# iSEE-Laboratory/DiffuVolume

Measured on AMD Instinct MI355X. Metric: stereo pairs/sec, SceneFlow 960x540 (cropped 960x512) maxdisp=192, hot path, higher is better.
Workload: dtype f32; 1 GPU; SceneFlow ACVNet+DiffuVolume hot path (gwc + concat*softmax(att) + 5 DDIM steps + EPE), 960x512, maxdisp=192, batch=8/GPU, random-init weights; global_batch=8, ddim_steps=5, parallelism=dp1

## Files before the change

### diffuvolume_amd/csrc/conv3d_s2pp.hip

```cpp

#include <atomic>
#include <type_traits>

#include "dv_common.h"

namespace {

typedef float f32x2 __attribute__((ext_vector_type(2)));

constexpr int kPPLoaders = 3;
constexpr int kPPDepth = 3;

template <int SHAPE_>
struct PG {
  static constexpr int SHAPE = SHAPE_;
  static_assert(SHAPE == 0 || SHAPE == 1, "patch shapes");
  static constexpr int TR = SHAPE == 0 ? 2 : 4, TC = 16 / TR;
  static constexpr int KC = 4, NT = 2, TD = 2;
  static constexpr int IZ = 2 * TD + 1, IY = 4 * TR + 1;
  static constexpr int LQ = SHAPE == 0 ? TC + 2 : TC + 1;
  static constexpr int RX = SHAPE == 0 ? 40 : 20;
  static constexpr int ROWS = IZ * IY;
  static constexpr int CS = ROWS * RX;
  static constexpr int QPC = ROWS * LQ;
  static constexpr int NQ = KC * QPC;
  static constexpr int NP = (NQ + 63) / 64;
  static constexpr int RAW_FLOATS = ((NP + 3) / 4 * 4) * 256;
  static_assert(RX == 4 * LQ && CS == 4 * QPC, "the loaded quads of a chunk are contiguous in LDS: quad `it` at float 4 * it");
  static_assert(4 * RAW_FLOATS * 4 <= 160 * 1024, "one block per CU: two sub-tiles x two bricks");
};

namespace pp {
constexpr int U_CHUNK = 3 * 4 * 4 * 4 * 16 * 4;
__host__ __device__ constexpr int amap(int i) { return i < 2 ? 0 : (i == 2 ? 1 : 2); }
__host__ __device__ constexpr int bmap(int i) { return i == 3 ? 1 : (i == 4 ? 3 : i); }
}

struct PPArgs {
  const float* in;
  const float* wpk;
  const float* ch_scale;
  const float* ch_bias;
  const float* residual;
  float* out;
  int B, Cin, D, H, W, Cout, Do, Ho, Wo;
  int ntx, nty, ntz, nco;
  int ntiles;
  int act;
  int vec_ok;
  unsigned wpk_bytes;
};

struct Tile { int tcb, z0, y0, x0, b; bool valid; };

template <int SHAPE>
__global__ __launch_bounds__(512 + 64 * kPPLoaders, 1) void conv3d_s2pp_kernel(PPArgs a) {
  using G = PG<SHAPE>;
  constexpr int KC = G::KC, NT = G::NT, TR = G::TR, TC = G::TC, IY = G::IY, RX = G::RX, CS = G::CS, LQ = G::LQ;
  constexpr int NQ = G::NQ, QPC = G::QPC, NP = G::NP, RAW_FLOATS = G::RAW_FLOATS;
  __shared__ __attribute__((aligned(16))) float raw_a0[RAW_FLOATS];
  __shared__ __attribute__((aligned(16))) float raw_b0[RAW_FLOATS];
  __shared__ __attribute__((aligned(16))) float raw_a1[RAW_FLOATS];
  __shared__ __attribute__((aligned(16))) float raw_b1[RAW_FLOATS];

  const int tid = threadIdx.x;
  const int lane = tid & 63;
  const int wave = __builtin_amdgcn_readfirstlane(tid >> 6);

  const unsigned nblk = gridDim.x, xcd = blockIdx.x & 7u, bidx = blockIdx.x >> 3;
  const unsigned nbx = (nblk >> 3) + (xcd < (nblk & 7u) ? 1u : 0u);
  const unsigned npairs = ((unsigned)a.ntiles + 1u) >> 1;
  const unsigned tq = npairs >> 3, trm = npairs & 7u;
  const unsigned slab_lo = xcd < trm ? xcd * (tq + 1) : trm * (tq + 1) + (xcd - trm) * tq;
  const unsigned slab_n = tq + (xcd < trm ? 1u : 0u);
  const int my_tiles = __builtin_amdgcn_readfirstlane(bidx < slab_n ? (int)((slab_n - bidx + nbx - 1) / nbx) : 0);
  if (my_tiles == 0) return;

  auto tile_at = [&](int k, int h) __attribute__((always_inline)) {
    unsigned t = 2u * (slab_lo + bidx + (unsigned)k * nbx) + (unsigned)h;
    Tile r;
    r.valid = t < (unsigned)a.ntiles;
    if (!r.valid) t = (unsigned)a.ntiles - 1u;
    r.tcb = t % a.nco; t /= a.nco;
    r.x0 = (t % a.ntx) * 2 * TC; t /= a.ntx;
    r.y0 = (t % a.nty) * 2 * TR; t /= a.nty;
    r.z0 = (t % a.ntz) * G::TD;
    r.b = t / a.ntz;
    return r;
  };

  const size_t plane = (size_t)a.H * a.W;
  const size_t vol = (size_t)a.D * plane;
  const unsigned vol_bytes = (unsigned)__builtin_amdgcn_readfirstlane((int)(vol * sizeof(float)));
  const int n_chunk = (a.Cin + KC - 1) / KC;
  const int NCH = (n_chunk + 1) & ~1;
  const bool share = (a.nco & 1) == 0;
  const int n_steps = my_tiles * NCH;

  if (wave >= 8) {
    constexpr int NL = kPPLoaders, NPL = (NP + NL - 1) / NL;
    const int li = wave - 8;
    static_assert(NL * NPL * 256 <= RAW_FLOATS, "every piece a loader writes lies inside the buffer");
    unsigned sob0[NPL], sob1[NPL];
    auto plan = [&](const Tile& t, unsigned (&sob)[NPL]) __attribute__((always_inline)) {
#pragma unroll
      for (int p = 0; p < NPL; ++p) {
        const int it = 64 * (li + NL * p) + lane;
        const int cl = it / QPC, r1 = it - cl * QPC;
        const int row = r1 / LQ, q = r1 - row * LQ;
        const int zz = row / IY, yy = row - zz * IY;
        const int z = 2 * t.z0 - 1 + zz, y = 2 * t.y0 - 1 + yy, x = 2 * t.x0 - 4 + 4 * q;
        const bool ok = t.valid && it < NQ && (unsigned)z < (unsigned)a.D && (unsigned)y < (unsigned)a.H &&
                        (unsigned)x < (unsigned)a.W;
        sob[p] = ok ? (unsigned)cl * vol_bytes + (unsigned)((z * a.H + y) * a.W + x) * 4u : 0xfffffff0u;
      }
    };
    auto dma_raw = [&](const Tile& t, const unsigned (&sob)[NPL], int c, float* dst) __attribute__((always_inline)) {
      const int c0 = c * KC;
      const int left = a.Cin - c0;
      const unsigned rec = left <= 0 ? 0u : (unsigned)(left < KC ? left : KC) * vol_bytes;
      const uint64_t ba = reinterpret_cast<uint64_t>(a.in + ((size_t)t.b * a.Cin + (left > 0 ? c0 : 0)) * vol);
      const uint64_t bu = (uint64_t)(unsigned)__builtin_amdgcn_readfirstlane((int)(unsigned)ba) |
                          ((uint64_t)(unsigned)__builtin_amdgcn_readfirstlane((int)(unsigned)(ba >> 32)) << 32);
      const auto rs = __builtin_amdgcn_make_buffer_rsrc(reinterpret_cast<float*>(bu), 0,
                                                        __builtin_amdgcn_readfirstlane((int)rec), 0x00020000);
#pragma unroll
      for (int p = 0; p < NPL; ++p)
        __builtin_amdgcn_raw_ptr_buffer_load_lds(rs, (__attribute__((address_space(3))) void*)(dst + (li + NL * p) * 256), 16,
                                                 (int)sob[p], 0, 0, 0);
    };
    Tile ft0 = tile_at(0, 0), ft1 = tile_at(0, 1);
    int fk = 0, fc = 0;
    auto advance = [&]() __attribute__((always_inline)) {
      if (++fc == NCH) {
        fc = 0;
        if (++fk < my_tiles) { ft0 = tile_at(fk, 0); ft1 = tile_at(fk, 1); plan(ft0, sob0); plan(ft1, sob1); }
      }
    };
    auto fetch = [&](float* d0, float* d1) __attribute__((always_inline)) {
      dma_raw(ft0, sob0, fc, d0);
      if (!share) dma_raw(ft1, sob1, fc, d1);
      advance();
    };
    plan(ft0, sob0);
    plan(ft1, sob1);
    fetch(raw_a0, raw_a1);
    fetch(raw_b0, raw_b1);
    auto arrive = [&]() __attribute__((always_inline)) {
      asm volatile("s_waitcnt vmcnt(0)" ::: "memory");
      __syncthreads();
    };
    arrive();
#pragma unroll 1
    for (int s = 0; s < n_steps; s += 2) {
      arrive();
      if (s + 2 < n_steps) fetch(raw_a0, raw_a1);
      arrive();
      if (s + 3 < n_steps) fetch(raw_b0, raw_b1);
    }
    return;
  }

  const int sub = wave >> 2, pl = (wave >> 1) & 1, nh = wave & 1;
  const int j = lane & 15, kq = lane >> 4;
  const float* const raw_a = (sub && !share) ? raw_a1 : raw_a0;
  const float* const raw_b = (sub && !share) ? raw_b1 : raw_b0;

  const uint64_t wb = reinterpret_cast<uint64_t>(a.wpk);
  const uint64_t wbs = (uint64_t)(unsigned)__builtin_amdgcn_readfirstlane((int)(unsigned)wb) |
                       ((uint64_t)(unsigned)__builtin_amdgcn_readfirstlane((int)(unsigned)(wb >> 32)) << 32);
  const auto wrs = __builtin_amdgcn_make_buffer_rsrc(reinterpret_cast<float*>(wbs), 0, (int)a.wpk_bytes, 0x00020000);
  const int wvoff = lane * 16;
  constexpr int PD = kPPDepth, RD = PD == 5 ? 6 : PD + 1;
  static_assert(12 % RD == 0, "ring slots repeat with the step");
  f32x4 bq[RD][NT];
  auto load_b = [&](int tcb, int chunk, int g, int slot) __attribute__((always_inline)) {
    const int ch = chunk < n_chunk ? chunk : n_chunk - 1;
    const int kd = g >> 2, by = g & 3;
    const int base = (ch * a.nco + tcb) * (pp::U_CHUNK * 4);
#pragma unroll
    for (int n = 0; n < NT; ++n) {
      const int so = base + (((kd * 4 + 2 * nh + n) * 4 + by) * 256) * 4;
      bq[slot][n] = __builtin_bit_cast(f32x4, __builtin_amdgcn_raw_buffer_load_b128(wrs, wvoff, so, 0));
    }
  };

  const int a_tr = j / TC, a_tc = j % TC;
  const int patch_lo = kq * CS + ((2 * pl) * IY + 4 * a_tr) * RX + 4 * a_tc;

  float V[2][5][5];
  auto read_row = [&](const float* rb, int kd, int slot, int r) __attribute__((always_inline)) {
    const float* p = rb + patch_lo + kd * IY * RX;
    V[slot][r][0] = p[r * RX + 3];
    const f32x4 qd = *reinterpret_cast<const f32x4*>(p + r * RX + 4);
    V[slot][r][1] = qd[0]; V[slot][r][2] = qd[1]; V[slot][r][3] = qd[2]; V[slot][r][4] = qd[3];
  };
  auto col_tf = [&](int slot, int r) __attribute__((always_inline)) {
    V[slot][r][0] -= V[slot][r][2];
    V[slot][r][4] -= V[slot][r][2];
  };
  auto row_tf = [&](int slot) __attribute__((always_inline)) {
#pragma unroll
    for (int c = 0; c < 5; ++c) {
      V[slot][0][c] -= V[slot][2][c];
      V[slot][4][c] -= V[slot][2][c];
    }
  };

  f32x4 acc[3][3][NT];
  auto zero_acc = [&]() __attribute__((always_inline)) {
#pragma unroll
    for (int i = 0; i < 3; ++i)
#pragma unroll
      for (int jj = 0; jj < 3; ++jj)
#pragma unroll
        for (int n = 0; n < NT; ++n) acc[i][jj][n] = (f32x4){0.f, 0.f, 0.f, 0.f};
  };

  const size_t oplane = (size_t)a.Ho * a.Wo;
  const float slope = a.act == DV_ACT_RELU ? 0.f : (a.act == DV_ACT_LEAKY ? 0.01f : 1.f);
  auto epilogue = [&](const Tile& t) __attribute__((always_inline)) {
    constexpr int RL = TC < 4 ? TC : 4, NRUN = 4 / RL;
    const int zo = t.z0 + pl;
    if (zo >= a.Do || !t.valid) return;
    const bool fast = a.vec_ok && t.x0 + 2 * TC <= a.Wo && t.y0 + 2 * TR <= a.Ho;
#pragma unroll
    for (int n = 0; n < NT; ++n) {
      const int co = t.tcb * 64 + nh * 32 + n * 16 + j;
      if (co >= a.Cout) continue;
      const float sc = a.ch_scale ? a.ch_scale[co] : 1.f;
      const float bi = a.ch_bias ? a.ch_bias[co] : 0.f;
      const size_t cbase = (((size_t)t.b * a.Cout + co) * a.Do + zo) * oplane;
#pragma unroll
      for (int run = 0; run < NRUN; ++run) {
        const int m0 = 4 * kq + run * RL;
        const int yo = t.y0 + 2 * (m0 / TC), xo = t.x0 + 2 * (m0 % TC);
#pragma unroll
        for (int ya = 0; ya < 2; ++ya) {
          float v[2 * RL];
#pragma unroll
          for (int e = 0; e < RL; ++e)
#pragma unroll
            for (int xb = 0; xb < 2; ++xb) {
              const int ee = run * RL + e;
              v[2 * e + xb] = (acc[ya][xb][n][ee] + acc[ya][xb + 1][n][ee]) + (acc[ya + 1][xb][n][ee] + acc[ya + 1][xb + 1][n][ee]);
            }
          const size_t o = cbase + (size_t)(yo + ya) * a.Wo + xo;
          if (fast) {
#pragma unroll
            for (int h = 0; h < RL / 2; ++h) {
              f32x4 u = (f32x4){v[4 * h], v[4 * h + 1], v[4 * h + 2], v[4 * h + 3]} * sc + bi;
              if (a.residual) u += *reinterpret_cast<const f32x4*>(a.residual + o + 4 * h);
              if (a.act == DV_ACT_MISH) {
#pragma unroll
                for (int e = 0; e < 4; ++e) u[e] = dv_act(u[e], DV_ACT_MISH);
              } else {
                u = __builtin_elementwise_max(u, u * slope);
              }
              *reinterpret_cast<f32x4*>(a.out + o + 4 * h) = u;
            }
          } else if (yo + ya < a.Ho) {
#pragma unroll
            for (int e = 0; e < 2 * RL; ++e)
              if (xo + e < a.Wo) {
                float u = fmaf(v[e], sc, bi);
                if (a.residual) u += a.residual[o + e];
                a.out[o + e] = dv_act(u, a.act);
              }
          }
        }
      }
    }
  };

  Tile cur = tile_at(0, sub);
  Tile nxt = my_tiles > 1 ? tile_at(1, sub) : cur;
#pragma unroll
  for (int g = 0; g < PD; ++g) load_b(cur.tcb, 0, g, g);
  zero_acc();
  __syncthreads();
#pragma unroll
  for (int r = 0; r < 5; ++r) read_row(raw_a, 0, 0, r);
  row_tf(0);
  col_tf(0, 0); col_tf(0, 2); col_tf(0, 4);

  auto step = [&](int c, auto parity) __attribute__((always_inline)) {
    constexpr int PAR = decltype(parity)::value;
    const float* rb = PAR ? raw_b : raw_a;
    const float* nb = PAR ? raw_a : raw_b;
    const bool n1 = c + 1 >= NCH;
    const int c1 = n1 ? 0 : c + 1;
    const int tcb1 = n1 ? nxt.tcb : cur.tcb;
#pragma unroll
    for (int g = 0; g < 12; ++g) {
      const int kd = g >> 2, by = g & 3;
      const int slot = (PAR + kd) & 1, nslot = slot ^ 1;
      if (g == 10) __syncthreads();
      if (g + PD < 12) load_b(cur.tcb, c, g + PD, (g + PD) % RD);
      else load_b(tcb1, c1, g + PD - 12, (g + PD) % RD);
      {
        const float* src = kd < 2 ? rb : nb;
        const int nkd = kd < 2 ? kd + 1 : 0;
        if (by == 0) { col_tf(slot, 1); col_tf(slot, 3); }
        if (by == 2) { read_row(src, nkd, nslot, 0); read_row(src, nkd, nslot, 2); read_row(src, nkd, nslot, 4); }
        if (by == 3) { read_row(src, nkd, nslot, 1); read_row(src, nkd, nslot, 3); }
      }
#pragma unroll
      for (int i = 0; i < 5; ++i) {
        if (pp::bmap(i) != by) continue;
#pragma unroll
        for (int jj = 0; jj < 5; ++jj)
#pragma unroll
          for (int n = 0; n < NT; ++n)
            acc[pp::amap(i)][pp::amap(jj)][n] = __builtin_amdgcn_mfma_f32_16x16x4f32(
                V[slot][i][jj], bq[g % RD][n][pp::bmap(jj)], acc[pp::amap(i)][pp::amap(jj)][n], 0, 0, 0);
      }
      if (by == 3) { row_tf(nslot); col_tf(nslot, 0); col_tf(nslot, 2); col_tf(nslot, 4); }
      __builtin_amdgcn_sched_barrier(0);
    }
  };

#pragma unroll 1
  for (int k = 0; k < my_tiles; ++k) {
#pragma unroll 1
    for (int c = 0; c < NCH; c += 2) {
      step(c, std::integral_constant<int, 0>{});
      step(c + 1, std::integral_constant<int, 1>{});
    }
    epilogue(cur);
    zero_acc();
    cur = nxt;
    if (k + 2 < my_tiles) nxt = tile_at(k + 2, sub);
  }
}

__global__ void pack_s2pp_weights_kernel(const float* __restrict__ w, float* __restrict__ wpk, int Cin, int Cout,
                                         int nchunk, int nco) {
  const size_t total = (size_t)nchunk * nco * 3 * 4 * 4 * 4 * 16;
  for (size_t i = (size_t)blockIdx.x * blockDim.x + threadIdx.x; i < total; i += (size_t)gridDim.x * blockDim.x) {
    size_t r = i;
    const int n = (int)(r % 16); r /= 16;
    const int k = (int)(r % 4); r /= 4;
    const int by = (int)(r % 4); r /= 4;
    const int nt = (int)(r % 4); r /= 4;
    const int kd = (int)(r % 3); r /= 3;
    const int cb = (int)(r % nco);
    const int ch = (int)(r / nco);
    const int co = cb * 64 + nt * 16 + n, ci = ch * 4 + k;
    double g[3][3];
    for (int p = 0; p < 3; ++p)
      for (int q = 0; q < 3; ++q)
        g[p][q] = (co < Cout && ci < Cin) ? (double)w[(((size_t)co * Cin + ci) * 3 + kd) * 9 + p * 3 + q] : 0.0;
    double row[3];
    for (int q = 0; q < 3; ++q) row[q] = by == 0 ? g[0][q] : (by == 1 ? g[1][q] : (by == 2 ? g[0][q] + g[2][q] : g[2][q]));
    float* dst = wpk + i * 4;
    dst[0] = (float)row[0];
    dst[1] = (float)row[1];
    dst[2] = (float)(row[0] + row[2]);
    dst[3] = (float)row[2];
  }
}

inline int cdiv(int a, int b) { return (a + b - 1) / b; }

int cu_count() {
  int dev = 0, v = 0;
  if (hipGetDevice(&dev) != hipSuccess) return 256;
  static std::atomic<int> cache[64];
  if (dev >= 0 && dev < 64 && (v = cache[dev].load(std::memory_order_relaxed)) > 0) return v;
  if (hipDeviceGetAttribute(&v, hipDeviceAttributeMultiprocessorCount, dev) != hipSuccess || v <= 0) return 256;
  if (dev >= 0 && dev < 64) cache[dev].store(v, std::memory_order_relaxed);
  return v;
}

}

extern "C" int dv_conv3d_s2pp_supported(int Cin, int Cout, int D, int H, int W) {
  return (Cin > 0 && Cout >= 64 && Cout % 64 == 0 && D > 0 && H > 0 && W > 0 && W % 4 == 0 &&
          (size_t)D * H * W * sizeof(float) <= 0x3fffffffull) ? 1 : 0;
}

extern "C" size_t dv_conv3d_s2pp_packed_floats(int Cin, int Cout) {
  if (Cin <= 0 || Cout <= 0) return 0;
  return (size_t)cdiv(Cin, 4) * cdiv(Cout, 64) * pp::U_CHUNK;
}

extern "C" int dv_conv3d_s2pp_pack_weights_f32(const float* w, float* wpacked, int Cin, int Cout, dv_stream_t stream) {
  DV_REQUIRE_PTR(w);
  DV_REQUIRE_PTR(wpacked);
  DV_REQUIRE(Cin > 0 && Cout > 0, DV_ERR_SHAPE);
  const int nchunk = cdiv(Cin, 4), nco = cdiv(Cout, 64);
  const size_t total = (size_t)nchunk * nco * 3 * 4 * 4 * 4 * 16;
  const int blocks = (int)((total + 255) / 256 < 4096 ? (total + 255) / 256 : 4096);
  hipLaunchKernelGGL(pack_s2pp_weights_kernel, dim3(blocks), dim3(256), 0, (hipStream_t)stream, w, wpacked, Cin, Cout,
                     nchunk, nco);
  return dv_launch_status();
}

extern "C" int dv_conv3d_s2pp_f32(const float* in, const float* wpacked, const float* ch_scale, const float* ch_bias,
                                  const float* residual, float* out, int B, int Cin, int D, int H, int W, int Cout,
                                  int act, dv_stream_t stream) {
  DV_REQUIRE_PTR(in);
  DV_REQUIRE_PTR(wpacked);
  DV_REQUIRE_PTR(out);
  DV_REQUIRE(B > 0 && Cin > 0 && D > 0 && H > 0 && W > 0 && Cout > 0, DV_ERR_SHAPE);
  DV_REQUIRE(dv_conv3d_s2pp_supported(Cin, Cout, D, H, W), DV_ERR_UNSUPPORTED);
  DV_REQUIRE(act >= DV_ACT_NONE && act <= DV_ACT_LEAKY, DV_ERR_UNSUPPORTED);
  DV_REQUIRE(dv_aligned16(wpacked) && dv_aligned16(in), DV_ERR_ALIGN);
  const size_t wbytes = dv_conv3d_s2pp_packed_floats(Cin, Cout) * sizeof(float);
  DV_REQUIRE(wbytes <= 0x7fffffffull, DV_ERR_SHAPE);
  PPArgs a;
  a.in = in; a.wpk = wpacked; a.ch_scale = ch_scale; a.ch_bias = ch_bias; a.residual = residual; a.out = out;
  a.B = B; a.Cin = Cin; a.D = D; a.H = H; a.W = W; a.Cout = Cout; a.act = act;
  a.Do = (D - 1) / 2 + 1; a.Ho = (H - 1) / 2 + 1; a.Wo = (W - 1) / 2 + 1;
  a.vec_ok = (a.Wo % 4 == 0) && dv_aligned16(out) && (!residual || dv_aligned16(residual));
  a.wpk_bytes = (unsigned)wbytes;
  hipStream_t s = (hipStream_t)stream;
  auto launch = [&](auto shape) {
    constexpr int SHAPE = decltype(shape)::value;
    using G = PG<SHAPE>;
    a.ntx = cdiv(a.Wo, 2 * G::TC); a.nty = cdiv(a.Ho, 2 * G::TR); a.ntz = cdiv(a.Do, G::TD); a.nco = cdiv(Cout, 64);
    const long long tiles = (long long)B * a.nco * a.ntz * a.nty * a.ntx;
    if (tiles <= 0 || tiles > 0x7fffffffLL) return (int)DV_ERR_SHAPE;
    a.ntiles = (int)tiles;
    const long long slots = cu_count();
    const long long pairs = (tiles + 1) / 2;
    const unsigned blocks = (unsigned)(pairs < slots ? pairs : slots);
    hipLaunchKernelGGL((conv3d_s2pp_kernel<SHAPE>), dim3(blocks), dim3(512 + 64 * kPPLoaders), 0, s, a);
    return dv_launch_status();
  };
  auto padded = [&](int tw, int th) { return (long long)cdiv(a.Wo, tw) * tw * cdiv(a.Ho, th) * th; };
  const int shape = padded(16, 4) < padded(8, 8) ? 0 : 1;
  if (shape == 1) return launch(std::integral_constant<int, 1>{});
  return launch(std::integral_constant<int, 0>{});
}
```

Baseline: 63.83 pairs/s.

## Stage per-channel scale/bias in LDS via loader wave and specialize plain epilogue

The loader wave 0 now writes each tile's per-channel scale and bias into a small 4-slot LDS ring, so the compute waves' epilogue reads them from LDS instead of global memory. A separate kernel instantiation without residual or Mish handling is launched when neither is needed. Lane ids become opaque asm values, the next tile is held only as its channel block index, and sched barriers and scalar LDS base addresses are added, all aimed at lowering register pressure and scalarising addresses in the MFMA loop. The ring depth and the extra lgkmcnt wait add a coupling between loader and compute progress, and the removed co<Cout guard assumes Cout is a multiple of 64.

New measurement: 64.17 pairs/s (median of 6 runs). Within noise of the previous version (+0.5%).

```diff
diff --git a/diffuvolume_amd/csrc/conv3d_s2pp.hip b/diffuvolume_amd/csrc/conv3d_s2pp.hip
--- a/diffuvolume_amd/csrc/conv3d_s2pp.hip
+++ b/diffuvolume_amd/csrc/conv3d_s2pp.hip
@@ -27,7 +27,7 @@
   static constexpr int NP = (NQ + 63) / 64;
   static constexpr int RAW_FLOATS = ((NP + 3) / 4 * 4) * 256;
   static_assert(RX == 4 * LQ && CS == 4 * QPC, "the loaded quads of a chunk are contiguous in LDS: quad `it` at float 4 * it");
-  static_assert(4 * RAW_FLOATS * 4 <= 160 * 1024, "one block per CU: two sub-tiles x two bricks");
+  static_assert(4 * RAW_FLOATS * 4 + 4096 <= 160 * 1024, "one block per CU: two sub-tiles x two bricks");
 };
 
 namespace pp {
@@ -51,10 +51,16 @@
   unsigned wpk_bytes;
 };
 
+__device__ __forceinline__ int opaque_lane() {
+  int ln;
+  asm volatile("v_mbcnt_lo_u32_b32 %0, -1, 0\n\tv_mbcnt_hi_u32_b32 %0, -1, %0" : "=v"(ln));
+  return ln;
+}
+
 struct Tile { int tcb, z0, y0, x0, b; bool valid; };
 
-template <int SHAPE>
-__global__ __launch_bounds__(512 + 64 * kPPLoaders, 1) void conv3d_s2pp_kernel(PPArgs a) {
+template <int SHAPE, bool PLAIN>
+__device__ __forceinline__ void conv3d_s2pp_body(const PPArgs& a) {
   using G = PG<SHAPE>;
   constexpr int KC = G::KC, NT = G::NT, TR = G::TR, TC = G::TC, IY = G::IY, RX = G::RX, CS = G::CS, LQ = G::LQ;
   constexpr int NQ = G::NQ, QPC = G::QPC, NP = G::NP, RAW_FLOATS = G::RAW_FLOATS;
@@ -62,10 +68,9 @@
   __shared__ __attribute__((aligned(16))) float raw_b0[RAW_FLOATS];
   __shared__ __attribute__((aligned(16))) float raw_a1[RAW_FLOATS];
   __shared__ __attribute__((aligned(16))) float raw_b1[RAW_FLOATS];
-
-  const int tid = threadIdx.x;
-  const int lane = tid & 63;
-  const int wave = __builtin_amdgcn_readfirstlane(tid >> 6);
+  __shared__ __attribute__((aligned(16))) float sb_s[4][2][128];
+
+  const int wave = __builtin_amdgcn_readfirstlane((int)threadIdx.x >> 6);
 
   const unsigned nblk = gridDim.x, xcd = blockIdx.x & 7u, bidx = blockIdx.x >> 3;
   const unsigned nbx = (nblk >> 3) + (xcd < (nblk & 7u) ? 1u : 0u);
@@ -100,6 +105,7 @@
   if (wave >= 8) {
     constexpr int NL = kPPLoaders, NPL = (NP + NL - 1) / NL;
     const int li = wave - 8;
+    const int lane = opaque_lane();
     static_assert(NL * NPL * 256 <= RAW_FLOATS, "every piece a loader writes lies inside the buffer");
     unsigned sob0[NPL], sob1[NPL];
     auto plan = [&](const Tile& t, unsigned (&sob)[NPL]) __attribute__((always_inline)) {
@@ -113,6 +119,7 @@
         const bool ok = t.valid && it < NQ && (unsigned)z < (unsigned)a.D && (unsigned)y < (unsigned)a.H &&
                         (unsigned)x < (unsigned)a.W;
         sob[p] = ok ? (unsigned)cl * vol_bytes + (unsigned)((z * a.H + y) * a.W + x) * 4u : 0xfffffff0u;
+        __builtin_amdgcn_sched_barrier(0);
       }
     };
     auto dma_raw = [&](const Tile& t, const unsigned (&sob)[NPL], int c, float* dst) __attribute__((always_inline)) {
@@ -124,17 +131,27 @@
                           ((uint64_t)(unsigned)__builtin_amdgcn_readfirstlane((int)(unsigned)(ba >> 32)) << 32);
       const auto rs = __builtin_amdgcn_make_buffer_rsrc(reinterpret_cast<float*>(bu), 0,
                                                         __builtin_amdgcn_readfirstlane((int)rec), 0x00020000);
+      unsigned d0 = (unsigned)(size_t)(__attribute__((address_space(3))) float*)(dst + li * 256);
+      asm volatile("" : "+s"(d0));
 #pragma unroll
       for (int p = 0; p < NPL; ++p)
-        __builtin_amdgcn_raw_ptr_buffer_load_lds(rs, (__attribute__((address_space(3))) void*)(dst + (li + NL * p) * 256), 16,
+        __builtin_amdgcn_raw_ptr_buffer_load_lds(rs, (__attribute__((address_space(3))) void*)(size_t)(d0 + NL * p * 1024), 16,
                                                  (int)sob[p], 0, 0, 0);
     };
     Tile ft0 = tile_at(0, 0), ft1 = tile_at(0, 1);
     int fk = 0, fc = 0;
+    auto put_sb = [&]() __attribute__((always_inline)) {
+      if (li != 0) return;
+      const int c0 = ft0.tcb * 64 + lane, c1 = ft1.tcb * 64 + lane;
+      const float s0 = a.ch_scale ? a.ch_scale[c0] : 1.f, s1 = a.ch_scale ? a.ch_scale[c1] : 1.f;
+      const float b0 = a.ch_bias ? a.ch_bias[c0] : 0.f, b1 = a.ch_bias ? a.ch_bias[c1] : 0.f;
+      float (&d)[2][128] = sb_s[fk & 3];
+      d[0][lane] = s0; d[0][64 + lane] = b0; d[1][lane] = s1; d[1][64 + lane] = b1;
+    };
     auto advance = [&]() __attribute__((always_inline)) {
       if (++fc == NCH) {
         fc = 0;
-        if (++fk < my_tiles) { ft0 = tile_at(fk, 0); ft1 = tile_at(fk, 1); plan(ft0, sob0); plan(ft1, sob1); }
+        if (++fk < my_tiles) { ft0 = tile_at(fk, 0); ft1 = tile_at(fk, 1); plan(ft0, sob0); plan(ft1, sob1); put_sb(); }
       }
     };
     auto fetch = [&](float* d0, float* d1) __attribute__((always_inline)) {
@@ -144,10 +161,11 @@
     };
     plan(ft0, sob0);
     plan(ft1, sob1);
+    put_sb();
     fetch(raw_a0, raw_a1);
     fetch(raw_b0, raw_b1);
     auto arrive = [&]() __attribute__((always_inline)) {
-      asm volatile("s_waitcnt vmcnt(0)" ::: "memory");
+      asm volatile("s_waitcnt vmcnt(0) lgkmcnt(0)" ::: "memory");
       __syncthreads();
     };
     arrive();
@@ -162,6 +180,7 @@
   }
 
   const int sub = wave >> 2, pl = (wave >> 1) & 1, nh = wave & 1;
+  const int lane = opaque_lane();
   const int j = lane & 15, kq = lane >> 4;
   const float* const raw_a = (sub && !share) ? raw_a1 : raw_a0;
   const float* const raw_b = (sub && !share) ? raw_b1 : raw_b0;
@@ -219,17 +238,21 @@
 
   const size_t oplane = (size_t)a.Ho * a.Wo;
   const float slope = a.act == DV_ACT_RELU ? 0.f : (a.act == DV_ACT_LEAKY ? 0.01f : 1.f);
-  auto epilogue = [&](const Tile& t) __attribute__((always_inline)) {
+  auto epilogue = [&](const Tile& t, int k) __attribute__((always_inline)) {
+    const int ln = opaque_lane();
+    const int j = ln & 15, kq = ln >> 4;
     constexpr int RL = TC < 4 ? TC : 4, NRUN = 4 / RL;
     const int zo = t.z0 + pl;
     if (zo >= a.Do || !t.valid) return;
     const bool fast = a.vec_ok && t.x0 + 2 * TC <= a.Wo && t.y0 + 2 * TR <= a.Ho;
+    const float* sb = sb_s[k & 3][sub] + nh * 32 + j;
+    float scn[NT], bin[NT];
+#pragma unroll
+    for (int n = 0; n < NT; ++n) { scn[n] = sb[n * 16]; bin[n] = sb[64 + n * 16]; }
 #pragma unroll
     for (int n = 0; n < NT; ++n) {
       const int co = t.tcb * 64 + nh * 32 + n * 16 + j;
-      if (co >= a.Cout) continue;
-      const float sc = a.ch_scale ? a.ch_scale[co] : 1.f;
-      const float bi = a.ch_bias ? a.ch_bias[co] : 0.f;
+      const float sc = scn[n], bi = bin[n];
       const size_t cbase = (((size_t)t.b * a.Cout + co) * a.Do + zo) * oplane;
 #pragma unroll
       for (int run = 0; run < NRUN; ++run) {
@@ -250,8 +273,8 @@
 #pragma unroll
             for (int h = 0; h < RL / 2; ++h) {
               f32x4 u = (f32x4){v[4 * h], v[4 * h + 1], v[4 * h + 2], v[4 * h + 3]} * sc + bi;
-              if (a.residual) u += *reinterpret_cast<const f32x4*>(a.residual + o + 4 * h);
-              if (a.act == DV_ACT_MISH) {
+              if (!PLAIN && a.residual) u += *reinterpret_cast<const f32x4*>(a.residual + o + 4 * h);
+              if (!PLAIN && a.act == DV_ACT_MISH) {
 #pragma unroll
                 for (int e = 0; e < 4; ++e) u[e] = dv_act(u[e], DV_ACT_MISH);
               } else {
@@ -264,8 +287,9 @@
             for (int e = 0; e < 2 * RL; ++e)
               if (xo + e < a.Wo) {
                 float u = fmaf(v[e], sc, bi);
-                if (a.residual) u += a.residual[o + e];
-                a.out[o + e] = dv_act(u, a.act);
+                if (!PLAIN && a.residual) u += a.residual[o + e];
+                a.out[o + e] = !PLAIN ? dv_act(u, a.act)
+                               : (a.act == DV_ACT_RELU ? dv_act(u, DV_ACT_RELU) : (a.act == DV_ACT_LEAKY ? dv_act(u, DV_ACT_LEAKY) : u));
               }
           }
         }
@@ -274,7 +298,7 @@
   };
 
   Tile cur = tile_at(0, sub);
-  Tile nxt = my_tiles > 1 ? tile_at(1, sub) : cur;
+  int nxt_tcb = my_tiles > 1 ? tile_at(1, sub).tcb : cur.tcb;
 #pragma unroll
   for (int g = 0; g < PD; ++g) load_b(cur.tcb, 0, g, g);
   zero_acc();
@@ -290,7 +314,7 @@
     const float* nb = PAR ? raw_a : raw_b;
     const bool n1 = c + 1 >= NCH;
     const int c1 = n1 ? 0 : c + 1;
-    const int tcb1 = n1 ? nxt.tcb : cur.tcb;
+    const int tcb1 = n1 ? nxt_tcb : cur.tcb;
 #pragma unroll
     for (int g = 0; g < 12; ++g) {
       const int kd = g >> 2, by = g & 3;
@@ -327,11 +351,23 @@
       step(c, std::integral_constant<int, 0>{});
       step(c + 1, std::integral_constant<int, 1>{});
     }
-    epilogue(cur);
+    epilogue(cur, k);
     zero_acc();
-    cur = nxt;
-    if (k + 2 < my_tiles) nxt = tile_at(k + 2, sub);
+    if (k + 1 < my_tiles) {
+      cur = tile_at(k + 1, sub);
+      nxt_tcb = k + 2 < my_tiles ? tile_at(k + 2, sub).tcb : cur.tcb;
+    }
   }
+}
+
+template <int SHAPE>
+__global__ __launch_bounds__(512 + 64 * kPPLoaders, 1) void conv3d_s2pp_kernel(PPArgs a) {
+  conv3d_s2pp_body<SHAPE, true>(a);
+}
+
+template <int SHAPE>
+__global__ __launch_bounds__(512 + 64 * kPPLoaders, 1) void conv3d_s2pp_res_kernel(PPArgs a) {
+  conv3d_s2pp_body<SHAPE, false>(a);
 }
 
 __global__ void pack_s2pp_weights_kernel(const float* __restrict__ w, float* __restrict__ wpk, int Cin, int Cout,
@@ -426,7 +462,10 @@
     const long long slots = cu_count();
     const long long pairs = (tiles + 1) / 2;
     const unsigned blocks = (unsigned)(pairs < slots ? pairs : slots);
-    hipLaunchKernelGGL((conv3d_s2pp_kernel<SHAPE>), dim3(blocks), dim3(512 + 64 * kPPLoaders), 0, s, a);
+    if (residual == nullptr && act != DV_ACT_MISH)
+      hipLaunchKernelGGL((conv3d_s2pp_kernel<SHAPE>), dim3(blocks), dim3(512 + 64 * kPPLoaders), 0, s, a);
+    else
+      hipLaunchKernelGGL((conv3d_s2pp_res_kernel<SHAPE>), dim3(blocks), dim3(512 + 64 * kPPLoaders), 0, s, a);
     return dv_launch_status();
   };
   auto padded = [&](int tw, int th) { return (long long)cdiv(a.Wo, tw) * tw * cdiv(a.Ho, th) * th; };
```
